# HKUST-Aerial-Robotics/FUEL

Measured on AMD Instinct MI355X. Metric: plan_cycles_per_sec, higher is better.
Workload: dtype u64 bit-planes / u16 (u32 beyond 255 voxels) exact squared distances / f32 ESDF / f64 log-odds and B-spline

## Files before the change

### fuel_amd/_lib.py

```python
import ctypes as C
import os

_HERE = os.path.dirname(os.path.abspath(__file__))
LIB_PATH = os.environ.get("FUELMI_LIB_PATH") or os.path.join(_HERE, "libfuelmi.so")
_LIB = None

K_INFLATE, K_ESDF_ZY, K_ESDF_X, K_FRONTIER, K_BSPLINE, K_INSERT, K_COUNT = range(7)


class FuelmiError(RuntimeError):
    pass


class MapCfg(C.Structure):
    _fields_ = [
        ("resolution", C.c_double),
        ("map_size", C.c_double * 3),
        ("ground_height", C.c_double),
        ("obstacles_inflation", C.c_double),
        ("local_bound_inflate", C.c_double),
        ("default_dist", C.c_double),
        ("optimistic", C.c_int),
        ("signed_dist", C.c_int),
        ("p_hit", C.c_double),
# ... 204 lines not shown
RENDER_HOST_NODE, RENDER_CUDA_NODE = 0, 1


class BsplineCfg(C.Structure):
    _fields_ = [(n, C.c_double) for n in
                ("ld_smooth", "ld_dist", "ld_feasi", "ld_start", "ld_end", "ld_guide", "ld_waypt",
                 "ld_view", "ld_time", "dist0", "max_vel", "max_acc", "wnl", "dlmin")] + \
               [("bspline_degree", C.c_int)]


_dp = C.POINTER(C.c_double)
_ip = C.POINTER(C.c_int)


class BsplineBatch(C.Structure):
    _fields_ = [
        ("cost_function", C.c_int), ("dim", C.c_int), ("point_num", C.c_int), ("n_traj", C.c_int),
        ("x", _dp), ("pt_dist", _dp), ("knot_span", _dp), ("time_lb", _dp),
        ("start_state", _dp), ("end_state", _dp), ("end_n", C.c_int),
        ("guide_pts", _dp), ("waypoints", _dp), ("waypt_idx", _ip), ("n_waypt", C.c_int),
        ("view_pt", _dp), ("view_dir", _dp), ("view_idx", _ip),
    ]


_P = C.c_void_p
_PP = C.POINTER(C.c_void_p)
SYMBOLS = {
    "fuelmi_last_error": (C.c_char_p, []),
    "fuelmi_version": (C.c_char_p, []),
    "fuelmi_init": (C.c_int, [C.c_int]),
    "fuelmi_hw_queues": (C.c_int, []),
    "fuelmi_hw_queues_state": (C.c_int, []),
    "fuelmi_device_count": (C.c_int, []),
    "fuelmi_map_create": (C.c_int, [C.POINTER(MapCfg), _PP]),
    "fuelmi_map_destroy": (None, [_P]),
    "fuelmi_map_get_info": (C.c_int, [_P, C.POINTER(MapInfo)]),
    "fuelmi_map_input_points": (C.c_int, [_P, C.c_void_p, C.c_int, C.c_int, _dp]),
    "fuelmi_map_insert_plan": (C.c_int, [_ip]),
    "fuelmi_map_input_depth": (C.c_int, [_P, C.c_void_p, C.c_int, C.c_int, C.POINTER(DepthCfg), _dp, _dp,
                                         C.POINTER(C.c_int)]),
    "fuelmi_host_register": (C.c_int, [C.c_void_p, C.c_size_t]),
    "fuelmi_host_unregister": (C.c_int, [C.c_void_p]),
    "fuelmi_device_alloc": (C.c_int, [C.c_int, C.c_size_t, C.POINTER(C.c_void_p)]),
    "fuelmi_device_upload": (C.c_int, [C.c_void_p, C.c_void_p, C.c_size_t]),
    "fuelmi_device_free": (C.c_int, [C.c_void_p]),
    "fuelmi_hbm_triad": (C.c_int, [C.c_int, C.c_size_t, C.c_int, _dp]),
    "fuelmi_hbm_expand": (C.c_int, [C.c_int, C.c_size_t, C.c_int, _dp]),
    "fuelmi_map_project_depth": (C.c_int, [_P, C.c_void_p, C.c_int, C.c_int, C.POINTER(DepthCfg), _dp, _dp,
                                           C.c_void_p, C.c_int, C.POINTER(C.c_int)]),
    "fuelmi_map_inflate_local": (C.c_int, [_P]),
    "fuelmi_map_update_esdf": (C.c_int, [_P]),
    "fuelmi_map_set_esdf_family": (C.c_int, [_P, C.c_int]),
    "fuelmi_map_last_esdf_family": (C.c_int, [_P]),
    "fuelmi_map_esdf_plan": (C.c_int, [_ip, _ip, _ip, C.c_int, C.c_int, _ip]),
    "fuelmi_map_last_inflate_kernel": (C.c_int, [_P]),
    "fuelmi_map_reset_buffer_all": (C.c_int, [_P]),
    "fuelmi_map_reset_buffer": (C.c_int, [_P, _dp, _dp]),
    "fuelmi_map_set_occupied": (C.c_int, [_P, _dp, C.c_int, C.c_int]),
    "fuelmi_map_get_local_bound": (C.c_int, [_P, _ip, _ip]),
    "fuelmi_map_set_local_bound": (C.c_int, [_P, _ip, _ip]),
    "fuelmi_map_get_updated_box": (C.c_int, [_P, _dp, _dp, C.c_int]),
    "fuelmi_map_set_updated_box": (C.c_int, [_P, _dp, _dp]),
    "fuelmi_map_upload_occupancy": (C.c_int, [_P, _dp]),
    "fuelmi_map_sync_host": (C.c_int, [_P, _ip, _ip, _dp, C.c_void_p, _dp]),
    "fuelmi_map_register_mirrors": (C.c_int, [_P, _dp, C.c_void_p, _dp]),
    "fuelmi_map_unregister_mirrors": (C.c_int, [_P]),
    "fuelmi_map_dist_grad": (C.c_int, [_P, _dp, C.c_int, _dp, _dp]),
    "fuelmi_map_coarse_dist": (C.c_int, [_P, _dp, C.c_int, _dp]),
    "fuelmi_map_query_state": (C.c_int, [_P, _ip, C.c_int, _ip, _ip]),
    "fuelmi_map_synchronize": (C.c_int, [_P]),
    "fuelmi_frontier_set_viewpoint_cfg": (C.c_int, [_P, C.POINTER(ViewpointCfg)]),
    "fuelmi_frontier_compute_to_visit": (C.c_int, [_P, C.POINTER(C.c_int), C.POINTER(C.c_int)]),
    "fuelmi_frontier_viewpoint_count": (C.c_int, [_P, C.c_int, C.c_int]),
    "fuelmi_frontier_viewpoints": (C.c_int, [_P, C.c_int, C.c_int, _dp, C.POINTER(C.c_int)]),
    "fuelmi_frontier_is_covered": (C.c_int, [_P, C.POINTER(C.c_int)]),
    "fuelmi_frontier_cluster_filtered_size": (C.c_int, [_P, C.c_int, C.c_int]),
    "fuelmi_frontier_cluster_filtered": (C.c_int, [_P, C.c_int, C.c_int, C.c_void_p]),
    "fuelmi_frontier_create": (C.c_int, [_P, C.POINTER(FrontierCfg), _PP]),
    "fuelmi_frontier_destroy": (None, [_P]),
    "fuelmi_frontier_reset": (C.c_int, [_P]),
    "fuelmi_frontier_stats": (C.c_int, [_P, C.POINTER(C.c_int)]),
    "fuelmi_frontier_resolved_in_launch": (C.c_int, [_P]),
    "fuelmi_frontier_path_stats": (C.c_int, [_P, C.POINTER(C.c_int)]),
    "fuelmi_frontier_changed_stats": (C.c_int, [_P, C.POINTER(C.c_int)]),
    "fuelmi_frontier_order_stats": (C.c_int, [_P, C.POINTER(C.c_int)]),
    "fuelmi_frontier_synchronize": (C.c_int, [_P]),
    "fuelmi_bench_cycles": (C.c_int, [_P, _P, _P, _dp, _dp, C.c_int, C.c_int, C.POINTER(C.c_int), _dp]),
    "fuelmi_bench_host_profile": (C.c_int, [_P, _dp]),
    "fuelmi_bench_cycles_delivered": (C.c_int, [_P, _P, _P, _dp, _dp, C.c_int, _ip, C.c_size_t, _dp, _dp,
                                                C.POINTER(C.c_int), _dp]),
    "fuelmi_bench_stream": (C.c_int, [_P, _P, _P, C.c_int, C.POINTER(C.c_void_p), C.c_int, C.c_int, C.POINTER(DepthCfg),
                                      _dp, _dp, C.c_int, C.POINTER(C.c_int), _dp, _dp]),
    "fuelmi_frontier_search": (C.c_int, [_P, _ip]),
    "fuelmi_frontier_search_begin": (C.c_int, [_P]),
    "fuelmi_frontier_search_end": (C.c_int, [_P, _ip]),
    "fuelmi_frontier_keep_previous": (C.c_int, [_P, C.c_int]),
    "fuelmi_frontier_commit": (C.c_int, [_P, C.c_int]),
    "fuelmi_frontier_count": (C.c_int, [_P, C.c_int]),
    "fuelmi_frontier_cluster_size": (C.c_int, [_P, C.c_int, C.c_int]),
    "fuelmi_frontier_cluster_cells": (C.c_int, [_P, C.c_int, C.c_int, _ip]),
    "fuelmi_frontier_cluster_centres": (C.c_int, [_P, C.c_int, C.c_int, _dp]),
    "fuelmi_frontier_cluster_info": (C.c_int, [_P, C.c_int, C.c_int, _dp]),
    "fuelmi_frontier_removed_count": (C.c_int, [_P]),
    "fuelmi_frontier_removed_ids": (C.c_int, [_P, _ip]),
    "fuelmi_frontier_get_flags": (C.c_int, [_P, C.c_void_p]),
    "fuelmi_map_path_costs": (C.c_int, [_P, C.POINTER(PathCfg), C.c_int, _dp, _dp, _dp, _ip, _ip, _dp]),
# ... 110 lines not shown
```

### fuel_amd/csrc/esdf.hip

```cpp
#include <algorithm>
#include <cmath>
#include <vector>

#include "fuelmi_internal.h"

template <int MODE>
__device__ __forceinline__ u64 src_word(const u64* __restrict__ infl, const u64* __restrict__ unk, long w) {
  if (MODE == 0) return infl[w] | unk[w];
  if (MODE == 1) return infl[w];
  return ~infl[w];
}

template <int MODE>
__device__ __forceinline__ int nearest_src(const u64* __restrict__ infl, const u64* __restrict__ unk,
                                           long linebit, int zlo, int zhi, int z) {
  int best = -1;
  {
    long pos = linebit + z, end = linebit + zhi;
    long w = pos >> 6;
    u64 word = src_word<MODE>(infl, unk, w) & (~0ull << (pos & 63));
    while (true) {
      if (word) {
        long c = (w << 6) + __builtin_ctzll(word);
        if (c <= end) best = (int)(c - pos);
// ... 969 lines not shown
    }
  }
}

template <int MODE, int GMAX, int NW>
__global__ void __launch_bounds__(1024)
k_esdf_zy_pk2(Geo g, Box3 b, const u64* __restrict__ infl, const u64* __restrict__ unk, uint4* __restrict__ tmp16,
              u32* __restrict__ wide, Pk2ZChunks ch, int z0a, int npx, int fastrow, u32* __restrict__ stat,
              u32* __restrict__ src_flag, u32 serial, unsigned long long* __restrict__ dbg) {
  extern __shared__ __attribute__((aligned(16))) unsigned char smem_raw[];
  const int nzc = ch.n;
  const int xcd = blockIdx.x & 7, slot = blockIdx.x >> 3;
  const int q = xcd + 8 * (slot / nzc);
  if (q >= npx) return;
  unsigned long long* stamp = dbg ? dbg + 8 * (size_t)blockIdx.x : nullptr;
  if (stamp && threadIdx.x == 0) stamp[0] = wall_clock64();
  const int c = slot % nzc;
  const int seg0 = ch.seg0[c], tile0 = ch.tile0[c], tstride = ch.tstride[c], gsh = ch.gsh[c], off = ch.off[c];
#define PK2_BODY(GG) zy_pk2_body<MODE, GG, NW>(g, b, infl, unk, tmp16, wide, z0a, seg0, tile0, tstride, gsh, off, npx, q, fastrow, stat, src_flag, serial, stamp, smem_raw)
  switch (ch.g[c]) {
    case 8:
      if constexpr (GMAX >= 8) PK2_BODY(8);
      break;
    case 4:
      if constexpr (GMAX >= 4) PK2_BODY(4);
      break;
    case 2: PK2_BODY(2); break;
    default: PK2_BODY(1); break;
  }
#undef PK2_BODY
}

__device__ __noinline__ u32 x_slow_col16(const u32* tile, int c, const u32* __restrict__ wide_col, long row_stride, int xlen, int row) {
  u32 best = INF32;
  const int rmax = max(row, xlen - 1 - row);
  for (int r = 0; r <= rmax && (u32)__mul24(r, r) < best; ++r) {
    const u32 rr = (u32)__mul24(r, r);
#pragma unroll
    for (int s = 0; s < 2; ++s) {
      const int qrow = s ? row + r : row - r;
      if (qrow < 0 || qrow >= xlen || (s && !r)) continue;
      u32 v = (tile[(qrow >> 1) * 32 + c] >> (16 * (qrow & 1))) & 0xffffu;
      if (v == PK_NOSRC) continue;
      if (v >= PK_INF) v = wide_col[(long)qrow * row_stride];
      best = min(best, v + rr);
    }
  }
  return best;
}

template <int OUT>
__global__ void __launch_bounds__(512)
k_esdf_x_pk2(Geo g, Box3 b, const uint4* __restrict__ tmp16, const u32* __restrict__ wide, float* __restrict__ dist, Pk2Chunks ch,
             int z0a, int full8, u32* stat, volatile u32* h_stat, const u32* __restrict__ src_flag, u32 serial,
             unsigned long long* __restrict__ dbg) {
  constexpr int SEGS = 8;
  extern __shared__ __attribute__((aligned(16))) unsigned char smem_raw[];
  forward_stat(stat, h_stat);
  uint4* tile = reinterpret_cast<uint4*>(smem_raw);
  const int xlen = b.hi[0] - b.lo[0] + 1;
  const int ylen = b.hi[1] - b.lo[1] + 1;
  const int npx = (xlen + 1) >> 1;
  const int T = blockDim.x;
  const int total = npx * SEGS;
  const float resf = (float)g.res;
  unsigned long long* stamp = dbg ? dbg + 8 * (size_t)blockIdx.x : nullptr;
  if (stamp && threadIdx.x == 0) stamp[0] = wall_clock64();
  int gw = 8, gsh = 3, y0, seg0, t;
  if ((int)blockIdx.x < full8) {
    const int xcd = blockIdx.x & 7, slot = blockIdx.x >> 3;
    y0 = xcd + 8 * (slot / ch.n8);
    if (y0 >= ylen) return;
    const int c8 = slot % ch.n8;
    seg0 = 8 * c8;
    t = y0 * ch.n8 + c8;
  } else {
    t = (int)blockIdx.x - full8 + ylen * ch.n8;
    int c = ch.n8;
    while (c + 1 < ch.n && t >= ch.tile0[c + 1]) ++c;
    gw = ch.g[c], gsh = gw == 4 ? 2 : (gw == 2 ? 1 : 0);
    y0 = (t - ch.tile0[c]) * (8 >> gsh);
    seg0 = ch.seg0[c];
  }
  const bool any_src = *src_flag == serial;
  if (any_src) {
    const uint4* src = tmp16 + pk2_index(t, 0, 0, npx);
#pragma unroll 4
    for (int o = threadIdx.x; o < total; o += T) tile[o] = src[o];
  }
  if (stamp && threadIdx.x == 0) stamp[1] = wall_clock64();
  __syncthreads();
  if (stamp && threadIdx.x == 0) stamp[2] = wall_clock64();
  int n_far = 0;
  for (int o = threadIdx.x; o < total; o += T) {
    const int p = o >> 3, seg = o & 7;
    const int yy = y0 + (seg >> gsh);
    if (yy >= ylen) continue;
    uint4 ra, rb;
    pk_scan8<SEGS, false>(smem_raw, p, seg, npx, xlen, any_src, false, n_far, ra, rb);
    const int z = z0a + 4 * (seg0 + (seg & (gw - 1)));
    const long coloff = (long)(b.lo[1] + yy) * g.nz + z;
    if (any_src && max(max4(ra.x, ra.y, ra.z, ra.w), max4(rb.x, rb.y, rb.z, rb.w)) >= PK_INF) {
      u32* pa = &ra.x;
      u32* pb = &rb.x;
      const u32* wc = wide + (long)b.lo[0] * g.nyz + coloff;
      for (int k = 0; k < 4; ++k) {
        if (pa[k] >= PK_INF) pa[k] = x_slow_col16(reinterpret_cast<const u32*>(smem_raw), 4 * seg + k, wc + k, g.nyz, xlen, 2 * p);
        if (2 * p + 1 < xlen && pb[k] >= PK_INF)
          pb[k] = x_slow_col16(reinterpret_cast<const u32*>(smem_raw), 4 * seg + k, wc + k, g.nyz, xlen, 2 * p + 1);
      }
    }
    float* dst = dist + (long)(b.lo[0] + 2 * p) * g.nyz + coloff;
    x_store4<OUT>(dst, z, b.lo[2], b.hi[2], ra, resf);
    if (2 * p + 1 < xlen) x_store4<OUT>(dst + g.nyz, z, b.lo[2], b.hi[2], rb, resf);
  }
  if (stamp && threadIdx.x == 0) stamp[3] = wall_clock64();
}


static hipError_t lds_attr_once(const void* fn, int bytes) {
  static std::mutex mu;
  static std::vector<std::pair<const void*, int>> done;
  int dev = 0;
  (void)hipGetDevice(&dev);
  std::lock_guard<std::mutex> lk(mu);
  for (const auto& d : done)
    if (d.first == fn && d.second == dev) return hipSuccess;
  const hipError_t e = hipFuncSetAttribute(fn, hipFuncAttributeMaxDynamicSharedMemorySize, bytes);
  if (e == hipSuccess) done.push_back({fn, dev});
  return e;
}

static int pass_timing_report(fuelmi_map* m, unsigned long long* dbg, int grid, const char* what) {
  HIPCHK(hipStreamSynchronize(m->stream));
  std::vector<unsigned long long> d((size_t)grid * 8);
// ... 74 lines not shown
      if (nz == PK2_MAXZCH) return false;
      zs->seg0[nz] = (short)(seg_lo + o), zs->g[nz] = (signed char)gz, zs->gsh[nz] = (signed char)gsh, zs->off[nz] = (signed char)o;
      zs->tile0[nz] = tile0, zs->tstride[nz] = tstride;
      ++nz;
    }
    return true;
  };
  for (int c = 0; c < n8; ++c, ++n, seg += 8) {
    if (n == PK2_MAXCH) return false;
    xs->seg0[n] = (short)seg, xs->g[n] = 8, xs->tile0[n] = 0;
    if (!add_z(seg, 8, 3, c, n8)) return false;
  }
  xs->n8 = n8;
  while (seg < nseg) {
    int gw = 4;
    while (gw > nseg - seg) gw >>= 1;
    const int gsh = gw == 4 ? 2 : (gw == 2 ? 1 : 0);
    if (n == PK2_MAXCH) return false;
    xs->seg0[n] = (short)seg, xs->g[n] = (short)gw, xs->tile0[n] = tile;
    if (!add_z(seg, gw, gsh, tile, 1)) return false;
    tile += (ylen + 8 / gw - 1) / (8 / gw);
    seg += gw;
    ++n;
  }
  xs->n = n;
  zs->n = nz;
  for (int k = n; k <= PK2_MAXCH; ++k) xs->tile0[k] = tile;
  for (int k = n; k < PK2_MAXCH; ++k) xs->g[k] = 1;
  if (n8 == n) xs->tile0[n8] = tile;
  return true;
}

size_t esdf_handover_bytes(int nx, int ny, int nz) {
  if (nz % 4 != 0) return 0;
  const size_t ntiles = ((size_t)ny * (size_t)((nz + 7) / 4 + 1) + 7) / 8 + PK2_MAXCH + 1;
  return ntiles * (size_t)(((nx + 1) / 2 + 63) / 64) * 64 * 128;
}

struct EsdfLaunch {
  int kernel = 0, targ[3] = {0, 0, 0};
  int grid = 0, block = 0, lds = 0;
  int ZC = 0, nzc = 0, z0a = 0;
  int aux = 0;
};
struct EsdfPlan {
  int n = 0;
  int family = 0;
  EsdfLaunch l[4];
  Pk2Chunks ch;
  Pk2ZChunks zch;
};

static int esdf_plan(const int dims[3], const Box3& b, int family, bool optimistic, bool signed_dist, size_t handover,
                     EsdfPlan* p) {
  *p = EsdfPlan{};
  const int xlen = b.hi[0] - b.lo[0] + 1, ylen = b.hi[1] - b.lo[1] + 1, zlen = b.hi[2] - b.lo[2] + 1;
  const int z0a = b.lo[2] & ~3, zlen_a = (b.hi[2] | 3) - z0a + 1;
  const int npx = (xlen + 1) >> 1, npair = (ylen + 1) >> 1;
  const bool z4 = dims[2] % 4 == 0;
  const int g_max = (size_t)npair * 4 * 32 > 52 * 1024 ? 2 : 4;
  const size_t pk2_lds = (size_t)npair * g_max * 32;
  const bool pk2 = z4 && zlen <= 255 && handover > 0 && (size_t)npx * 128 <= 150 * 1024 && pk2_lds <= 160 * 1024 - 64 &&
                   pk2_chunks(ylen, zlen_a >> 2, g_max, &p->ch, &p->zch) &&
                   (size_t)p->ch.tile0[p->ch.n] * npx * 128 <= handover;
  const bool vec4 = z4 && (size_t)xlen * 64 <= 150 * 1024;

  auto pass = [&](int fam, int mode, EsdfLaunch* L, int* ran) {
    const int out = mode == 2;
    EsdfLaunch& zy = L[0];
    EsdfLaunch& x = L[1];
    if (fam == FUELMI_ESDF_PLAIN && pk2) {
      zy = {FUELMI_ESDF_K_ZY_PK2, {mode, g_max, zlen_a > 128 ? 4 : 2}, ((npx + 7) / 8) * 8 * p->zch.n,
            2 * std::min(256, std::max(64, ((npair / 2 + 63) / 64) * 64)), (int)pk2_lds, 0, p->zch.n, z0a, npx};
      const int x_lds = npx * 8 * 16;
      const int full8 = ((ylen + 7) / 8) * 8 * p->ch.n8;
      x = {FUELMI_ESDF_K_X_PK2, {out, 0, 0}, full8 + (p->ch.tile0[p->ch.n] - ylen * p->ch.n8), x_lds > 32 * 1024 ? 512 : 256,
           x_lds, 0, p->ch.n, z0a, full8};
      *ran = FUELMI_ESDF_PLAIN;
      return FUELMI_OK;
    }
    const bool far = fam == FUELMI_ESDF_FAR;
    *ran = far ? FUELMI_ESDF_FAR : FUELMI_ESDF_PLAIN32;
    if (vec4) {
      const int budget = std::min(std::max(32 * 1024, ylen * 4 * 20), 80 * 1024);
      int zc_max = std::max(4, (budget / (4 * ylen)) & ~3);
      zc_max = std::min(zc_max, std::min(zlen_a, 64));
      int nzc = (zlen_a + zc_max - 1) / zc_max;
      const int ZC = (((zlen_a + nzc - 1) / nzc) + 3) & ~3;
      nzc = (zlen_a + ZC - 1) / ZC;
      auto zy_lds = [&](bool f) { return (size_t)(f ? ylen + ((ylen + 7) >> 3) + 1 : ylen) * ZC * sizeof(u32); };
      const bool zy_far = far && zy_lds(true) <= 160 * 1024;
      if (zy_lds(zy_far) > 160 * 1024) {
        fuelmi_set_error("ESDF y-line of %d voxels does not fit the LDS tile", ylen);
        return FUELMI_ELIMIT;
      }
      zy = {FUELMI_ESDF_K_ZY4, {mode, zy_far, 0}, ((xlen + 7) / 8) * 8 * nzc, 512, (int)zy_lds(zy_far), ZC, nzc, z0a, 0};
      const int segs = (size_t)xlen * 128 > 150 * 1024 ? 4 : 8;
      auto x_lds = [&](bool f) { return (size_t)(f ? xlen + ((xlen + 7) >> 3) + 1 : xlen) * segs * 4 * sizeof(u32); };
      const bool x_far = far && x_lds(true) <= 160 * 1024;
      x = {FUELMI_ESDF_K_X4, {out, segs, x_far}, (ylen * zlen_a + 4 * segs - 1) / (4 * segs), 1024, (int)x_lds(x_far), 0, 0,
           z0a, zlen_a};
      return FUELMI_OK;
    }
    const int zc_max = std::min(std::min(std::max(1, (16 * 1024) / (2 * ylen)), zlen), 256);
    const int nzc = (zlen + zc_max - 1) / zc_max;
    const int ZC = (zlen + nzc - 1) / nzc;
    const size_t lds = (size_t)ylen * ZC * sizeof(unsigned short);
    if (lds > 160 * 1024) {
      fuelmi_set_error("ESDF y-line of %d voxels does not fit the LDS tile", ylen);
      return FUELMI_ELIMIT;
    }
    zy = {FUELMI_ESDF_K_ZY, {mode, 0, 0}, xlen * nzc, 256, (int)lds, ZC, nzc, 0, 0};
    const int S = (size_t)xlen * 32 * 4 <= 64 * 1024 ? 32 : ((size_t)xlen * 16 * 4 <= 128 * 1024 ? 16 : ((size_t)xlen * 8 * 4 <= 128 * 1024 ? 8 : 0));
    if (!S) {
      fuelmi_set_error("ESDF x-line of %d voxels does not fit the LDS tile", xlen);
      return FUELMI_ELIMIT;
    }
    x = {FUELMI_ESDF_K_X, {S, out, 0}, (ylen * zlen + S - 1) / S, 256, xlen * S * (int)sizeof(u32), 0, 0, 0, 0};
    return FUELMI_OK;
  };

  int rc = pass(family, optimistic ? 1 : 0, &p->l[0], &p->family);
  if (rc) return rc;
  p->n = 2;
  if (signed_dist) {
    int ran;
    rc = pass(family == FUELMI_ESDF_FAR ? FUELMI_ESDF_PLAIN : family, 2, &p->l[2], &ran);
    if (rc) return rc;
    p->n = 4;
  }
// ... 66 lines not shown
  if (L.kernel == FUELMI_ESDF_K_ZY4) {
    auto go = [&](auto kern) {
      return esdf_launch(m, kern, L, 160 * 1024, g, b, infl, unk, m->esdf_tmp, L.ZC, L.nzc, L.z0a, ESDF_NEAR | (ZY_FASTROW << 8), stat);
    };
    if constexpr (MODE != 2)
      if (L.targ[1]) return go(&k_esdf_zy4<MODE, true>);
    return go(&k_esdf_zy4<MODE, false>);
  }
  const u32 serial = pk2_next_serial(m);
  return timed_launch(m, L, [&](unsigned long long* dbg) {
    auto go = [&](auto kern) {
      return esdf_launch(m, kern, L, 160 * 1024, g, b, infl, unk, reinterpret_cast<uint4*>(m->esdf_tmp16), m->esdf_tmp,
                         p.zch, L.z0a, L.aux, ZY_FASTROW, stat, pk2_src_flag(m), serial, dbg);
    };
    const bool g4 = L.targ[1] == 4, nw4 = L.targ[2] == 4;
    return g4 ? (nw4 ? go(&k_esdf_zy_pk2<MODE, 4, 4>) : go(&k_esdf_zy_pk2<MODE, 4, 2>))
              : (nw4 ? go(&k_esdf_zy_pk2<MODE, 2, 4>) : go(&k_esdf_zy_pk2<MODE, 2, 2>));
  });
}

template <int OUT>
static int launch_x(fuelmi_map* m, const Box3& b, const EsdfPlan& p, const EsdfLaunch& L) {
  const Geo& g = m->g;
  u32* stat = OUT == 0 ? m->esdf_stat : nullptr;
  if (L.kernel == FUELMI_ESDF_K_X) {
    auto go = [&](auto kern) { return esdf_launch(m, kern, L, 160 * 1024, g, b, (const u32*)m->esdf_tmp, m->dist); };
    return L.targ[0] == 32 ? go(&k_esdf_x<32, OUT>) : (L.targ[0] == 16 ? go(&k_esdf_x<16, OUT>) : go(&k_esdf_x<8, OUT>));
  }
  if (L.kernel == FUELMI_ESDF_K_X4) {
    auto go = [&](auto kern) {
      return esdf_launch(m, kern, L, 160 * 1024, g, b, (const u32*)m->esdf_tmp, m->dist, L.z0a, L.aux, ESDF_NEAR, stat,
                         esdf_stat_host(m));
    };
    const bool segs8 = L.targ[1] == 8;
    if constexpr (OUT == 0)
      if (L.targ[2]) return segs8 ? go(&k_esdf_x4<OUT, 8, true>) : go(&k_esdf_x4<OUT, 4, true>);
    return segs8 ? go(&k_esdf_x4<OUT, 8, false>) : go(&k_esdf_x4<OUT, 4, false>);
  }
  return timed_launch(m, L, [&](unsigned long long* dbg) {
    return esdf_launch(m, &k_esdf_x_pk2<OUT>, L, 150 * 1024, g, b, reinterpret_cast<const uint4*>(m->esdf_tmp16),
                       (const u32*)m->esdf_tmp, m->dist, p.ch, L.z0a, L.aux, stat, esdf_stat_host(m),
                       (const u32*)pk2_src_flag(m), m->esdf_serial, dbg);
  });
}

static bool esdf_is_zy(const EsdfLaunch& L) { return L.kernel <= FUELMI_ESDF_K_ZY_PK2; }


int esdf_update(fuelmi_map* m) {
  const Box3& b = m->local_bound;
  const int fam = m->esdf_family_pin >= 0 ? m->esdf_family_pin : (esdf_use_far(m, b) ? FUELMI_ESDF_FAR : FUELMI_ESDF_PLAIN);
  const int dims[3] = {m->g.nx, m->g.ny, m->g.nz};
  EsdfPlan p;
  int rc = esdf_plan(dims, b, fam, m->cfg.optimistic != 0, m->cfg.signed_dist != 0, m->esdf_tmp16_bytes, &p);
  if (rc) return rc;
  m->esdf_family_last = p.family;
  for (int i = 0; i < p.n && rc == FUELMI_OK; ++i) {
    const EsdfLaunch& L = p.l[i];
    StageScope sc(m, esdf_is_zy(L) ? FUELMI_K_ESDF_ZY : FUELMI_K_ESDF_X, nullptr, true);
    if (esdf_is_zy(L))
      rc = L.targ[0] == 0 ? launch_zy<0>(m, b, p, L) : (L.targ[0] == 1 ? launch_zy<1>(m, b, p, L) : launch_zy<2>(m, b, p, L));
    else
      rc = (L.kernel == FUELMI_ESDF_K_X ? L.targ[1] : L.targ[0]) == 0 ? launch_x<0>(m, b, p, L) : launch_x<1>(m, b, p, L);
  }
  return rc;
}

extern "C" int fuelmi_map_esdf_plan(const int dims[3], const int lo[3], const int hi[3], int family, int flags,
                                    int out[FUELMI_ESDF_PLAN_INTS]) {
  ARGCHK(dims && lo && hi && out && family >= FUELMI_ESDF_PLAIN && family <= FUELMI_ESDF_PLAIN32);
  Box3 b;
  for (int i = 0; i < 3; ++i) {
    ARGCHK(dims[i] > 0 && 0 <= lo[i] && lo[i] <= hi[i] && hi[i] < dims[i]);
    b.lo[i] = lo[i], b.hi[i] = hi[i];
  }
  EsdfPlan p;
  const int rc = esdf_plan(dims, b, family, (flags & FUELMI_ESDF_PLAN_OPTIMISTIC) != 0, (flags & FUELMI_ESDF_PLAN_SIGNED) != 0,
                           esdf_handover_bytes(dims[0], dims[1], dims[2]), &p);
  if (rc) return rc;
  for (int k = 0; k < FUELMI_ESDF_PLAN_INTS; ++k) out[k] = 0;
  out[0] = p.n, out[1] = p.family;
  for (int i = 0; i < p.n; ++i) {
    const EsdfLaunch& L = p.l[i];
    const int v[10] = {L.kernel, L.targ[0], L.targ[1], L.targ[2], L.grid, L.block, L.lds, L.ZC, L.nzc, L.z0a};
    for (int k = 0; k < 10; ++k) out[2 + 10 * i + k] = v[k];
  }
  return FUELMI_OK;
}

extern "C" int fuelmi_map_set_esdf_family(fuelmi_map* m, int family) {
  ARGCHK(m && family >= FUELMI_ESDF_AUTO && family <= FUELMI_ESDF_PLAIN32);
  m->esdf_family_pin = family;
  return FUELMI_OK;
}
extern "C" int fuelmi_map_last_esdf_family(const fuelmi_map* m) {
  ARGCHK(m);
  return m->esdf_family_last;
}
```

### fuel_amd/csrc/fuelmi_internal.h

```cpp
#ifndef FUELMI_INTERNAL_H_
#define FUELMI_INTERNAL_H_

#include <hip/hip_runtime.h>
#include <hip/hip_ext.h>

#include <atomic>
#include <cstdint>
#include <cstdio>
#include <condition_variable>
#include <cstdlib>
#include <memory>
#include <mutex>
#include <shared_mutex>
#include <thread>
#include <string>
#include <vector>

#include "../../include/fuelmi.h"

typedef unsigned long long u64;
typedef unsigned int u32;

void fuelmi_set_error(const char* fmt, ...);
#define HIPCHK(expr)                                                                        \
// ... 53 lines not shown
  signed char g[PK2_MAXZCH];
  signed char gsh[PK2_MAXZCH];
  signed char off[PK2_MAXZCH];
  int tile0[PK2_MAXZCH];
  int tstride[PK2_MAXZCH];
};

struct ProfileSlot {
  std::vector<hipEvent_t> ev;
  size_t used = 0;
};

struct fuelmi_map {
  fuelmi_map_cfg cfg;
  fuelmi_map_info info;
  Geo g;
  int device = 0;
  hipStream_t stream = nullptr;
  int margin_words = 0;

  double* occ = nullptr;
  Plane occ_bits;
  Plane unk_bits;
  Plane infl_bits;
  Plane tmp_bits;
  Plane tmp2_bits;
  float* dist = nullptr;
  u32* esdf_tmp = nullptr;
  u32* esdf_tmp16 = nullptr;
  size_t esdf_tmp16_bytes = 0;
  u32 esdf_serial = 0;
  unsigned char* flag_rayend = nullptr;
  u32* ray_owner = nullptr;
  Plane hit_bits, miss_bits;
  u64* ins_partial = nullptr;
  size_t ins_partial_cap = 0;
  struct Dependent {
    void* obj;
    void (*orphan)(void*);
  };
  std::vector<Dependent> dependents;
  std::mutex dep_mu;
  void* ins_rec = nullptr;
  size_t ins_rec_cap = 0;
  u64* ins_head = nullptr;
  u64* h_ins = nullptr;
  u64 ins_epoch = 0;
  u32* esdf_stat = nullptr;
  u32* h_esdf_stat = nullptr;
  u32 far_hist[256][2] = {};
  unsigned short far_tag[256] = {};
  bool far_last = false;
  int esdf_family_pin = FUELMI_ESDF_AUTO;
  int esdf_family_last = FUELMI_ESDF_PLAIN;
  signed char raycast_num = 0;
  unsigned occ_epoch = 0;

  Box3 local_bound;
  double upd_min[3], upd_max[3];
  bool reset_updated_box = true;

  std::mutex qmu;
  struct Mirror {
    void* host = nullptr;
    void* dev = nullptr;
  } mirror[3];
  void* d_stage = nullptr;
  size_t d_stage_bytes = 0;
  void* h_stage = nullptr;
  size_t h_stage_bytes = 0;

  struct QuerySlot {
    hipStream_t st = nullptr;
    hipEvent_t ev_dep = nullptr, ev_done = nullptr, ev_rd = nullptr;
    unsigned char* pin = nullptr;
    size_t pin_cap = 0;
    bool busy = false;
  };
  std::vector<std::unique_ptr<QuerySlot>> qslots;
  std::mutex qs_mu;
  std::condition_variable qs_cv;
  std::shared_timed_mutex rw_mu;
  std::mutex prof_mu;

  double bench_host_us[7] = {0, 0, 0, 0, 0, 0, 0};
  hipEvent_t t0 = nullptr, t1 = nullptr;
  int last_inflate_kernel = -1;
  hipEvent_t t_prof0 = nullptr;
  hipEvent_t ev_planes = nullptr;
  unsigned long long planes_ver = 0;
  std::vector<hipEvent_t> planes_read_evs;
  struct LateReader {
    hipStream_t st;
    hipEvent_t ev;
    bool* sticky;
  };
  std::vector<LateReader> late_readers;
  DevScratch path_dev;
  DevScratch refine_dev;
  DevScratch goal_dev;
  DevScratch kino_dev;
  DevScratch trajchk_dev;
  DevScratch trajsmp_dev;
  DevScratch trajadj_dev;
  DevScratch cloud_dev;
  DevScratch topo_dev;
// ... 268 lines not shown
```

### fuel_amd/host.py

```python
import ctypes as C

import numpy as np

from . import _lib
from ._lib import (BsplineBatch, BsplineCfg, CloudCfg, ColRangeCfg, FrontierCfg, GainCfg, GoalCfg, KinoCfg, LocalSegCfg, MapCfg, MapInfo, PathCfg, RefineCfg, RenderCfg, TopoCfg, TrajAdjCfg, TrajChkCfg, TrajSmpCfg, TspCfg,
                   WptrajCfg, YawCfg, YawPathCfg, check, lib)

DEFAULT_MAP = dict(resolution=0.1, ground_height=-1.0, obstacles_inflation=0.199,
                   local_bound_inflate=0.5, default_dist=0.0, optimistic=0, signed_dist=0,
                   p_hit=0.65, p_miss=0.35, p_min=0.12, p_max=0.90, p_occ=0.80,
                   max_ray_length=4.5, virtual_ceil_height=-10.0)
DEFAULT_BSPLINE = dict(ld_smooth=20.0, ld_dist=10.0, ld_feasi=2.0, ld_start=100.0, ld_end=0.5,
                       ld_guide=1.5, ld_waypt=0.3, ld_view=0.0, ld_time=1.0, dist0=0.7,
                       max_vel=2.0, max_acc=2.0, wnl=1.0, dlmin=0.0, bspline_degree=3)

SMOOTHNESS, DISTANCE, FEASIBILITY, START, END, GUIDE, WAYPOINTS, VIEWCONS, MINTIME = \
    (1 << k for k in range(9))
GUIDE_PHASE = SMOOTHNESS | GUIDE | START | END
NORMAL_PHASE = SMOOTHNESS | DISTANCE | FEASIBILITY | START | END


def _dp(a):
    return None if a is None else a.ctypes.data_as(C.POINTER(C.c_double))

# ... 221 lines not shown
    args = (_ip(o["status"]), _dp(o["duration"]), _ip(o["seg_num"]), _dp(o["dt_yaw"]), _dp(o["yaw_ctrl"]),
            _ip(o["n_waypt"]), _dp(o["waypts"]), _dp(o["end_yaw"]), _dp(o["cost"]), _dp(o["yawdot_ctrl"]),
            _dp(o["yawddot_ctrl"]))
    return o, args


def _d3(v):
    return (C.c_double * 3)(*[float(x) for x in v])


def _i3(v):
    return (C.c_int * 3)(*[int(x) for x in v])


class SDFMap:
    UNKNOWN, FREE, OCCUPIED = 0, 1, 2
    ESDF_AUTO, ESDF_PLAIN, ESDF_FAR, ESDF_PLAIN32 = -1, 0, 1, 2
    default_esdf_family = None

    def __init__(self, map_size, box_min=None, box_max=None, device=0, **params):
        self.L = lib()
        p = dict(DEFAULT_MAP)
        p.update(params)
        c = MapCfg()
        for k, v in p.items():
            setattr(c, k, v)
        org = (-map_size[0] / 2.0, -map_size[1] / 2.0, p["ground_height"])
        bmin = box_min if box_min is not None else org
        bmax = box_max if box_max is not None else tuple(org[i] + map_size[i] for i in range(3))
        for i in range(3):
            c.map_size[i] = float(map_size[i])
            c.box_min[i] = float(bmin[i])
            c.box_max[i] = float(bmax[i])
        c.device = device
        self.cfg = c
        h = C.c_void_p()
        check(self.L.fuelmi_map_create(C.byref(c), C.byref(h)))
        self.h = h
        info = MapInfo()
        check(self.L.fuelmi_map_get_info(self.h, C.byref(info)))
        self.info = info
        self.nvox = tuple(info.voxel_num)
        self.N = self.nvox[0] * self.nvox[1] * self.nvox[2]
        self.origin = np.array(info.origin)
        self.res = c.resolution
        if SDFMap.default_esdf_family is not None:
            self.setEsdfFamily(SDFMap.default_esdf_family)

    def setEsdfFamily(self, family):
        check(self.L.fuelmi_map_set_esdf_family(self.h, int(family)))

    def lastEsdfFamily(self):
        return self.L.fuelmi_map_last_esdf_family(self.h)

    _ESDF_KERNELS = (("k_esdf_zy", 1, None), ("k_esdf_zy4", 2, 1), ("k_esdf_zy_pk2", 3, None), ("k_esdf_x", 2, None),
                     ("k_esdf_x4", 3, 2), ("k_esdf_x_pk2", 1, None))

    @staticmethod
    def esdfPlan(dims, lo, hi, family, optimistic=False, signed_dist=False):
        out = (C.c_int * 42)()
        ints = lambda v: (C.c_int * 3)(*[int(a) for a in v])
        flags = (1 if optimistic else 0) | (2 if signed_dist else 0)
        check(lib().fuelmi_map_esdf_plan(ints(dims), ints(lo), ints(hi), int(family), flags, out))
        launches = []
        for i in range(out[0]):
            k, a0, a1, a2, grid, block, lds, zc, nzc, z0a = out[2 + 10 * i:12 + 10 * i]
            kname, nt, far = SDFMap._ESDF_KERNELS[k]
            targs = [("true" if a else "false") if j == far else str(a) for j, a in enumerate((a0, a1, a2)[:nt])]
            name = "%s<%s>" % (kname, ", ".join(targs))
            launches.append({"kernel": name, "grid": grid, "block": block, "lds": lds, "ZC": zc, "nzc": nzc, "z0a": z0a})
        return {"family": out[1], "launches": launches}

    @staticmethod
    def insertPlan():
        out = (C.c_int * 8)()
        check(lib().fuelmi_map_insert_plan(out))
        return {"lanes_per_ray": out[0], "ray_slots": out[1], "classify_slots": out[2], "cube": (out[3], out[4], out[5])}

    def lastInflateKernel(self):
        return self.L.fuelmi_map_last_inflate_kernel(self.h)

    def close(self):
        if getattr(self, "h", None):
            self.L.fuelmi_map_destroy(self.h)
            self.h = None

    def __del__(self):
        try:
            self.close()
        except Exception:
            pass

    def inputPointCloud(self, points, camera_pos):
        pts = np.ascontiguousarray(points, dtype=np.float32).reshape(-1, 3)
        check(self.L.fuelmi_map_input_points(self.h, pts.ctypes.data, 12, len(pts), _d3(camera_pos)))

    @staticmethod
    def depthConfig(fx=387.229248046875, fy=387.229248046875, cx=321.04638671875, cy=243.44969177246094,
                    maxdist=5.0, mindist=0.2, margin=2, scaling=1000.0, skip=2):
        return _lib.DepthCfg(fx, fy, cx, cy, maxdist, mindist, margin, scaling, skip)

    def inputDepthImage(self, depth, camera_pos, camera_q_wxyz, cfg=None):
        img = np.ascontiguousarray(depth, dtype=np.uint16)
        cfg = cfg or self.depthConfig()
        n = C.c_int(0)
        q = (C.c_double * 4)(*[float(v) for v in camera_q_wxyz])
# ... 1255 lines not shown
```

### include/fuelmi.h

```cpp
#ifndef FUELMI_H_
#define FUELMI_H_

#include <stddef.h>
#include <stdint.h>

#ifdef __cplusplus
extern "C" {
#endif

#define FUELMI_OK 0
#define FUELMI_EINVAL (-1)
#define FUELMI_ENODEV (-2)
#define FUELMI_EHIP (-3)
#define FUELMI_ENOMEM (-4)
#define FUELMI_ELIMIT (-5)

#define FUELMI_HWQ_UNINIT 0
#define FUELMI_HWQ_SET 1
#define FUELMI_HWQ_ENV 2
#define FUELMI_HWQ_LATE 3
int fuelmi_init(int hw_queues);
int fuelmi_hw_queues(void);
int fuelmi_hw_queues_state(void);
const char* fuelmi_last_error(void);
// ... 11 lines not shown
  int optimistic;
  int signed_dist;
  double p_hit, p_miss, p_min, p_max, p_occ;
  double max_ray_length;
  double virtual_ceil_height;
  double box_min[3], box_max[3];
  int device;
} fuelmi_map_cfg;

typedef struct {
  int voxel_num[3];
  double origin[3];
  double min_boundary[3], max_boundary[3];
  double resolution_inv;
  int box_min[3], box_max[3];
  double prob_hit_log, prob_miss_log, clamp_min_log, clamp_max_log, min_occupancy_log;
  int inflate_step;
} fuelmi_map_info;

typedef struct fuelmi_map fuelmi_map;

int fuelmi_map_create(const fuelmi_map_cfg* cfg, fuelmi_map** out);
void fuelmi_map_destroy(fuelmi_map* m);
int fuelmi_map_get_info(const fuelmi_map* m, fuelmi_map_info* info);

int fuelmi_map_input_points(fuelmi_map* m, const float* xyz, int stride_bytes, int n,
                            const double camera_pos[3]);
int fuelmi_map_insert_plan(int out[8]);
typedef struct {
  double fx, fy, cx, cy;
  double depth_filter_maxdist, depth_filter_mindist;
  int depth_filter_margin;
  double k_depth_scaling_factor;
  int skip_pixel;
} fuelmi_depth_cfg;
int fuelmi_host_register(void* ptr, size_t bytes);
int fuelmi_host_unregister(void* ptr);
int fuelmi_device_alloc(int device, size_t bytes, void** out);
int fuelmi_device_upload(void* dst, const void* src, size_t bytes);
int fuelmi_device_free(void* ptr);
int fuelmi_hbm_triad(int device, size_t bytes, int reps, double* gb_per_s);
int fuelmi_hbm_expand(int device, size_t bytes_in, int reps, double* gb_per_s);
int fuelmi_map_input_depth(fuelmi_map* m, const unsigned short* depth, int rows, int cols,
                           const fuelmi_depth_cfg* cfg, const double cam_pos[3], const double cam_q_wxyz[4],
                           int* n_points);
int fuelmi_map_project_depth(fuelmi_map* m, const unsigned short* depth, int rows, int cols,
                             const fuelmi_depth_cfg* cfg, const double cam_pos[3], const double cam_q_wxyz[4],
                             float* xyz, int cap, int* n_points);
int fuelmi_map_inflate_local(fuelmi_map* m);
int fuelmi_map_update_esdf(fuelmi_map* m);
enum { FUELMI_ESDF_AUTO = -1, FUELMI_ESDF_PLAIN = 0, FUELMI_ESDF_FAR = 1, FUELMI_ESDF_PLAIN32 = 2 };
int fuelmi_map_set_esdf_family(fuelmi_map* m, int family);
int fuelmi_map_last_esdf_family(const fuelmi_map* m);
enum {
  FUELMI_ESDF_K_ZY = 0,
  FUELMI_ESDF_K_ZY4 = 1,
  FUELMI_ESDF_K_ZY_PK2 = 2,
  FUELMI_ESDF_K_X = 3,
  FUELMI_ESDF_K_X4 = 4,
  FUELMI_ESDF_K_X_PK2 = 5
};
enum { FUELMI_ESDF_PLAN_OPTIMISTIC = 1, FUELMI_ESDF_PLAN_SIGNED = 2, FUELMI_ESDF_PLAN_INTS = 42 };
int fuelmi_map_esdf_plan(const int dims[3], const int lo[3], const int hi[3], int family, int flags,
                         int out[FUELMI_ESDF_PLAN_INTS]);
int fuelmi_map_last_inflate_kernel(const fuelmi_map* m);
int fuelmi_map_reset_buffer_all(fuelmi_map* m);
int fuelmi_map_reset_buffer(fuelmi_map* m, const double min_pos[3], const double max_pos[3]);
int fuelmi_map_set_occupied(fuelmi_map* m, const double* pos_xyz, int n, int occ);
int fuelmi_map_get_local_bound(const fuelmi_map* m, int bmin[3], int bmax[3]);
int fuelmi_map_set_local_bound(fuelmi_map* m, const int bmin[3], const int bmax[3]);
int fuelmi_map_get_updated_box(fuelmi_map* m, double bmin[3], double bmax[3], int reset);
int fuelmi_map_set_updated_box(fuelmi_map* m, const double bmin[3], const double bmax[3]);

int fuelmi_map_upload_occupancy(fuelmi_map* m, const double* occ);

int fuelmi_map_sync_host(fuelmi_map* m, const int bmin[3], const int bmax[3], double* occupancy,
                         char* inflate, double* distance);
int fuelmi_map_register_mirrors(fuelmi_map* m, double* occupancy, char* inflate, double* distance);
int fuelmi_map_unregister_mirrors(fuelmi_map* m);

int fuelmi_map_dist_grad(fuelmi_map* m, const double* pos_xyz, int n, double* dist, double* grad_xyz);
int fuelmi_map_coarse_dist(fuelmi_map* m, const double* pos_xyz, int n, double* dist);
int fuelmi_map_query_state(fuelmi_map* m, const int* idx_xyz, int n, int* occupancy, int* inflate);

int fuelmi_map_synchronize(fuelmi_map* m);

typedef struct {
  int cluster_min;
  double min_z;
  double cluster_size_xy;
  int down_sample;
  int split;
  int reference_order;
} fuelmi_frontier_cfg;

typedef struct fuelmi_frontier fuelmi_frontier;

int fuelmi_frontier_create(fuelmi_map* m, const fuelmi_frontier_cfg* cfg, fuelmi_frontier** out);
void fuelmi_frontier_destroy(fuelmi_frontier* f);
int fuelmi_frontier_reset(fuelmi_frontier* f);
int fuelmi_frontier_stats(const fuelmi_frontier* f, int out3[3]);
int fuelmi_frontier_resolved_in_launch(const fuelmi_frontier* f);
int fuelmi_frontier_path_stats(const fuelmi_frontier* f, int out2[2]);
int fuelmi_frontier_changed_stats(const fuelmi_frontier* f, int out[9]);
int fuelmi_frontier_order_stats(const fuelmi_frontier* f, int out4[4]);
int fuelmi_frontier_synchronize(fuelmi_frontier* f);
// ... 523 lines not shown
```

Baseline: 11400.

## Add grouped y-block ordering for packed ESDF x-pass on large boxes

```diff
diff --git a/fuel_amd/_lib.py b/fuel_amd/_lib.py
--- a/fuel_amd/_lib.py
+++ b/fuel_amd/_lib.py
@@ -280,6 +280,8 @@
     "fuelmi_map_update_esdf": (C.c_int, [_P]),
     "fuelmi_map_set_esdf_family": (C.c_int, [_P, C.c_int]),
     "fuelmi_map_last_esdf_family": (C.c_int, [_P]),
+    "fuelmi_map_set_esdf_x_order": (C.c_int, [_P, C.c_int]),
+    "fuelmi_map_last_esdf_x_order": (C.c_int, [_P]),
     "fuelmi_map_esdf_plan": (C.c_int, [_ip, _ip, _ip, C.c_int, C.c_int, _ip]),
     "fuelmi_map_last_inflate_kernel": (C.c_int, [_P]),
     "fuelmi_map_reset_buffer_all": (C.c_int, [_P]),
diff --git a/fuel_amd/csrc/esdf.hip b/fuel_amd/csrc/esdf.hip
--- a/fuel_amd/csrc/esdf.hip
+++ b/fuel_amd/csrc/esdf.hip
@@ -1045,7 +1045,7 @@
 template <int OUT>
 __global__ void __launch_bounds__(512)
 k_esdf_x_pk2(Geo g, Box3 b, const uint4* __restrict__ tmp16, const u32* __restrict__ wide, float* __restrict__ dist, Pk2Chunks ch,
-             int z0a, int full8, u32* stat, volatile u32* h_stat, const u32* __restrict__ src_flag, u32 serial,
+             int z0a, int nseg, u32* stat, volatile u32* h_stat, const u32* __restrict__ src_flag, u32 serial,
              unsigned long long* __restrict__ dbg) {
   constexpr int SEGS = 8;
   extern __shared__ __attribute__((aligned(16))) unsigned char smem_raw[];
@@ -1060,20 +1060,49 @@
   unsigned long long* stamp = dbg ? dbg + 8 * (size_t)blockIdx.x : nullptr;
   if (stamp && threadIdx.x == 0) stamp[0] = wall_clock64();
   int gw = 8, gsh = 3, y0, seg0, t;
-  if ((int)blockIdx.x < full8) {
-    const int xcd = blockIdx.x & 7, slot = blockIdx.x >> 3;
-    y0 = xcd + 8 * (slot / ch.n8);
-    if (y0 >= ylen) return;
-    const int c8 = slot % ch.n8;
-    seg0 = 8 * c8;
-    t = y0 * ch.n8 + c8;
+  if (nseg == 0) {
+    const int full8 = ((ylen + 7) >> 3) * 8 * ch.n8;
+    if ((int)blockIdx.x < full8) {
+      const int xcd = blockIdx.x & 7, slot = blockIdx.x >> 3;
+      y0 = xcd + 8 * (slot / ch.n8);
+      if (y0 >= ylen) return;
+      const int c8 = slot % ch.n8;
+      seg0 = 8 * c8;
+      t = y0 * ch.n8 + c8;
+    } else {
+      t = (int)blockIdx.x - full8 + ylen * ch.n8;
+      int c = ch.n8;
+      while (c + 1 < ch.n && t >= ch.tile0[c + 1]) ++c;
+      gw = ch.g[c], gsh = gw == 4 ? 2 : (gw == 2 ? 1 : 0);
+      y0 = (t - ch.tile0[c]) * (8 >> gsh);
+      seg0 = ch.seg0[c];
+    }
   } else {
-    t = (int)blockIdx.x - full8 + ylen * ch.n8;
-    int c = ch.n8;
-    while (c + 1 < ch.n && t >= ch.tile0[c + 1]) ++c;
-    gw = ch.g[c], gsh = gw == 4 ? 2 : (gw == 2 ? 1 : 0);
-    y0 = (t - ch.tile0[c]) * (8 >> gsh);
-    seg0 = ch.seg0[c];
+    const int q8 = (int)gridDim.x >> 3, r8 = (int)gridDim.x & 7, xcd = blockIdx.x & 7;
+    const int v = xcd * q8 + min(xcd, r8) + (int)(blockIdx.x >> 3);
+    const int G = v / nseg;
+    int j = v - G * nseg;
+    if (j < 8 * ch.n8) {
+      y0 = 8 * G + j / ch.n8;
+      if (y0 >= ylen) return;
+      const int c8 = j % ch.n8;
+      seg0 = 8 * c8;
+      t = y0 * ch.n8 + c8;
+    } else {
+      j -= 8 * ch.n8;
+      int c = ch.n8;
+      for (; c < ch.n; ++c) {
+        const int rows = 8 / ch.g[c];
+        const int cnt = min((int)ch.g[c], (ylen - 8 * G + rows - 1) / rows);
+        if (j < cnt) break;
+        j -= cnt;
+      }
+      if (c >= ch.n) return;
+      gw = ch.g[c], gsh = gw == 4 ? 2 : (gw == 2 ? 1 : 0);
+      t = ch.tile0[c] + G * gw + j;
+      y0 = (G * gw + j) * (8 >> gsh);
+      seg0 = ch.seg0[c];
+    }
   }
   const bool any_src = *src_flag == serial;
   if (any_src) {
@@ -1254,7 +1283,7 @@
 };
 
 static int esdf_plan(const int dims[3], const Box3& b, int family, bool optimistic, bool signed_dist, size_t handover,
-                     EsdfPlan* p) {
+                     int x_order, EsdfPlan* p) {
   *p = EsdfPlan{};
   const int xlen = b.hi[0] - b.lo[0] + 1, ylen = b.hi[1] - b.lo[1] + 1, zlen = b.hi[2] - b.lo[2] + 1;
   const int z0a = b.lo[2] & ~3, zlen_a = (b.hi[2] | 3) - z0a + 1;
@@ -1276,8 +1305,9 @@
             2 * std::min(256, std::max(64, ((npair / 2 + 63) / 64) * 64)), (int)pk2_lds, 0, p->zch.n, z0a, npx};
       const int x_lds = npx * 8 * 16;
       const int full8 = ((ylen + 7) / 8) * 8 * p->ch.n8;
+      const bool groups = x_order >= 0 ? x_order != 0 : (size_t)xlen * ylen * zlen_a * 6 > ((size_t)256 << 20);
       x = {FUELMI_ESDF_K_X_PK2, {out, 0, 0}, full8 + (p->ch.tile0[p->ch.n] - ylen * p->ch.n8), x_lds > 32 * 1024 ? 512 : 256,
-           x_lds, 0, p->ch.n, z0a, full8};
+           x_lds, 0, p->ch.n, z0a, groups ? zlen_a >> 2 : 0};
       *ran = FUELMI_ESDF_PLAIN;
       return FUELMI_OK;
     }
@@ -1450,9 +1480,10 @@
   const int fam = m->esdf_family_pin >= 0 ? m->esdf_family_pin : (esdf_use_far(m, b) ? FUELMI_ESDF_FAR : FUELMI_ESDF_PLAIN);
   const int dims[3] = {m->g.nx, m->g.ny, m->g.nz};
   EsdfPlan p;
-  int rc = esdf_plan(dims, b, fam, m->cfg.optimistic != 0, m->cfg.signed_dist != 0, m->esdf_tmp16_bytes, &p);
+  int rc = esdf_plan(dims, b, fam, m->cfg.optimistic != 0, m->cfg.signed_dist != 0, m->esdf_tmp16_bytes, m->esdf_x_order_pin, &p);
   if (rc) return rc;
   m->esdf_family_last = p.family;
+  m->esdf_x_order_last = p.l[1].kernel == FUELMI_ESDF_K_X_PK2 ? (p.l[1].aux != 0) : -1;
   for (int i = 0; i < p.n && rc == FUELMI_OK; ++i) {
     const EsdfLaunch& L = p.l[i];
     StageScope sc(m, esdf_is_zy(L) ? FUELMI_K_ESDF_ZY : FUELMI_K_ESDF_X, nullptr, true);
@@ -1474,7 +1505,7 @@
   }
   EsdfPlan p;
   const int rc = esdf_plan(dims, b, family, (flags & FUELMI_ESDF_PLAN_OPTIMISTIC) != 0, (flags & FUELMI_ESDF_PLAN_SIGNED) != 0,
-                           esdf_handover_bytes(dims[0], dims[1], dims[2]), &p);
+                           esdf_handover_bytes(dims[0], dims[1], dims[2]), FUELMI_ESDF_X_AUTO, &p);
   if (rc) return rc;
   for (int k = 0; k < FUELMI_ESDF_PLAN_INTS; ++k) out[k] = 0;
   out[0] = p.n, out[1] = p.family;
@@ -1491,6 +1522,15 @@
   m->esdf_family_pin = family;
   return FUELMI_OK;
 }
+extern "C" int fuelmi_map_set_esdf_x_order(fuelmi_map* m, int order) {
+  ARGCHK(m && order >= FUELMI_ESDF_X_AUTO && order <= FUELMI_ESDF_X_GROUPS);
+  m->esdf_x_order_pin = order;
+  return FUELMI_OK;
+}
+extern "C" int fuelmi_map_last_esdf_x_order(const fuelmi_map* m) {
+  ARGCHK(m);
+  return m->esdf_x_order_last;
+}
 extern "C" int fuelmi_map_last_esdf_family(const fuelmi_map* m) {
   ARGCHK(m);
   return m->esdf_family_last;
diff --git a/fuel_amd/csrc/fuelmi_internal.h b/fuel_amd/csrc/fuelmi_internal.h
--- a/fuel_amd/csrc/fuelmi_internal.h
+++ b/fuel_amd/csrc/fuelmi_internal.h
@@ -129,6 +129,8 @@
   unsigned short far_tag[256] = {};
   bool far_last = false;
   int esdf_family_pin = FUELMI_ESDF_AUTO;
+  int esdf_x_order_pin = FUELMI_ESDF_X_AUTO;
+  int esdf_x_order_last = -1;
   int esdf_family_last = FUELMI_ESDF_PLAIN;
   signed char raycast_num = 0;
   unsigned occ_epoch = 0;
diff --git a/fuel_amd/host.py b/fuel_amd/host.py
--- a/fuel_amd/host.py
+++ b/fuel_amd/host.py
@@ -297,6 +297,14 @@
 
     def lastEsdfFamily(self):
         return self.L.fuelmi_map_last_esdf_family(self.h)
+
+    ESDF_X_AUTO, ESDF_X_ROWS, ESDF_X_GROUPS = -1, 0, 1
+
+    def setEsdfXOrder(self, order):
+        check(self.L.fuelmi_map_set_esdf_x_order(self.h, int(order)))
+
+    def lastEsdfXOrder(self):
+        return self.L.fuelmi_map_last_esdf_x_order(self.h)
 
     _ESDF_KERNELS = (("k_esdf_zy", 1, None), ("k_esdf_zy4", 2, 1), ("k_esdf_zy_pk2", 3, None), ("k_esdf_x", 2, None),
                      ("k_esdf_x4", 3, 2), ("k_esdf_x_pk2", 1, None))
diff --git a/include/fuelmi.h b/include/fuelmi.h
--- a/include/fuelmi.h
+++ b/include/fuelmi.h
@@ -87,6 +87,9 @@
 enum { FUELMI_ESDF_AUTO = -1, FUELMI_ESDF_PLAIN = 0, FUELMI_ESDF_FAR = 1, FUELMI_ESDF_PLAIN32 = 2 };
 int fuelmi_map_set_esdf_family(fuelmi_map* m, int family);
 int fuelmi_map_last_esdf_family(const fuelmi_map* m);
+enum { FUELMI_ESDF_X_AUTO = -1, FUELMI_ESDF_X_ROWS = 0, FUELMI_ESDF_X_GROUPS = 1 };
+int fuelmi_map_set_esdf_x_order(fuelmi_map* m, int order);
+int fuelmi_map_last_esdf_x_order(const fuelmi_map* m);
 enum {
   FUELMI_ESDF_K_ZY = 0,
   FUELMI_ESDF_K_ZY4 = 1,
```

New measurement: 11290. 1.0% lower.
